# mueller-franzes/medfusion

Measured on AMD Instinct MI355X. Metric: images/sec at 256x256, 150 DDIM steps (DiffusionPipeline.sample incl. VAE decode), higher is better.
Workload: dtype f32 (emulated: fp16 pairs -- 23-bit operands, and 23-bit STORAGE of the tensors between the UNet's conv blocks: they exist as fp16 pairs only)

## Files before the change

medfusion_amd/csrc/conv_f16x2.hip:

```cpp
#include "common.h"
#include <string.h>
#include <mutex>
#include <vector>
#include "gn_partial.h"
#include "conv_plan.h"
#include "conv_f16x2.h"
#include "conv_f16x2_halo.h"
#include "conv_f16x2_group.h"
#include "winograd.h"

using namespace mf;

namespace {

struct Tile2 { int id, BM, BN, WM, WN, NST, HG; };
const Tile2 kTiles2[] = {
    {31, 128, 256, 2, 4, 3, 0}, {32, 256, 128, 4, 2, 3, 0}, {33, 128, 128, 2, 4, 3, 0}, {34, 128, 128, 4, 2, 3, 0}, {35, 256, 64, 4, 2, 3, 0},
    {36, 128, 64, 4, 2, 3, 0}, {37, 64, 256, 1, 8, 3, 0},
    {51, 128, 128, 2, 2, 2, 0}, {52, 128, 128, 2, 2, 3, 0}, {53, 64, 128, 2, 2, 3, 0}, {54, 128, 64, 2, 2, 3, 0},
    {61, 256, 128, 4, 2, 3, 6}, {62, 256, 128, 4, 2, 3, 7}, {63, 128, 128, 2, 4, 3, 4}, {64, 128, 128, 2, 4, 3, 5},
};
inline size_t tile_lds(const Tile2& t) {
  return t.HG ? (size_t)2 * t.HG * (t.WM * t.WN) * 1024 + (size_t)3 * t.BN * 128 : (size_t)t.NST * (t.BM + t.BN) * 128;
}
// ... 272 lines not shown
  if (pl.splitk > 1 && !(tree_possible(d, pl) && epilogue_stats_ok(d, pl, G)))
    return stats_lds_bytes(d->Cout / stats_slices(d->N, HW, d->Cout, G)) <= 64 * 1024 ? stats_chunks(HW) : 0;
  if (!epilogue_stats_ok(d, pl, G)) return 0;
  return HW >= pl.t.BM ? HW / pl.t.BM : 1;
}


}

namespace mf {
int f16x2_gn_parts(const MfConvDesc* d, int G) {
  Plan2 p2;
  return make_plan2(d, &p2) == MF_OK ? gn_parts2(d, p2, G) : 0;
}
size_t f16x2_workspace_bytes(const MfConvDesc* d) {
  Plan2 p2;
  if (make_plan2(d, &p2) != MF_OK || !p2.ok || p2.splitk <= 1) return 0;
  const size_t slabs = (size_t)p2.splitk * p2.M * d->Cout * sizeof(float);
  const size_t tree = tree_possible(d, p2) ? tree_handoff_bytes(d, p2) : 0;
  return slabs > tree ? slabs : tree;
}
}

#if MFC2_HZ & (256 | 512)
static float* g_conv_dbg = nullptr;
extern "C" void mf_debug_set_conv_dump(float* p) { g_conv_dbg = p; }
#endif

extern "C" {

int mf_conv2d_f16x2_ok(const MfConvDesc* d) {
  Plan2 pl;
  return d && pair_precision(d->precision) && make_plan2(d, &pl) == MF_OK && pl.ok ? 1 : 0;
}

static int bound_slots2(const MfConvDesc* d, const Plan2& pl, bool with_stats) {
  const int HW = pl.Hout * pl.Wout;
  if (pl.splitk == 1 || tree_possible(d, pl)) {
    if (!tile_sample_aligned(pl)) return 0;
    const int nw = pl.t.WM * pl.t.WN;
    return HW >= pl.t.BM ? (HW / pl.t.BM) * (d->Cout / pl.t.BN) * nw : (d->Cout / pl.t.BN) * (nw * HW / pl.t.BM);
  }
  if (with_stats) return 0;
  const long p4 = (long)HW * d->Cout / 4;
  int bx = (int)((p4 + 255) / 256);
  const int cap = cdiv(2048, d->N);
  if (bx > cap) bx = cap;
// ... 329 lines not shown
```

medfusion_amd/csrc/conv_f16x2_wino.inc:

```

static void wino_gemm_desc(const MfConvDesc* d, MfConvDesc* g) {
  *g = *d;
  g->N = 16 * d->N;
  g->Hin = 1;
  g->Win = (d->Hin / 2) * (d->Win / 2);
  g->KH = g->KW = 1;
  g->stride = 1;
  g->pad = 0;
  g->upsample = 3;
}
static bool wino_shape_ok(const MfConvDesc* d) {
  return d && d->precision == MF_CONV_FP32_F16X2 && d->KH == 3 && d->KW == 3 && d->stride == 1 && d->pad == 1 && d->upsample == 0 &&
         d->in_layout == MF_LAYOUT_NHWC && d->out_layout == MF_LAYOUT_NHWC && d->N > 0 && d->Hin >= 2 && d->Win >= 2 && d->Hin % 2 == 0 && d->Win % 2 == 0 &&
         d->C1 > 0 && d->C1 % 32 == 0 && d->C2 >= 0 && d->C2 % 32 == 0 && d->Cout % 64 == 0 && d->Cout <= 1024 && 256 % (d->Cout / 4) == 0 &&
         (double)d->N * 16.0 * (d->Hin / 2) * (d->Win / 2) < 2147483647.0;
}
static size_t wino_m_bytes(const MfConvDesc* d) {
  const size_t b = (size_t)16 * d->N * (d->Hin / 2) * (d->Win / 2) * d->Cout * sizeof(float);
  return (b + 255) & ~(size_t)255;
}
static bool wino_plan(const MfConvDesc* d, MfConvDesc* g, Plan2* pl) {
  if (!wino_shape_ok(d)) return false;
  wino_gemm_desc(d, g);
  if (make_plan2(g, pl) != MF_OK || !pl->ok) return false;
// ... 93 lines not shown
  const size_t mbytes = wino_m_bytes(d), need = mf_wino_workspace_bytes(d);
  MF_REQUIRE(workspace_bytes >= need, MF_EWORKSPACE, "conv_wino: workspace %zu < %zu", workspace_bytes, need);
  float* m = reinterpret_cast<float*>(workspace);
  int rc = conv_f16x2_prepare(v1s, v2s, us, nullptr, m, v1_bound, v2_bound, u_bound, nullptr, reinterpret_cast<char*>(workspace) + mbytes,
                              workspace_bytes - mbytes, sync, nullptr, 0, nullptr, &g, nullptr, &q, true);
  if (rc) return rc;
  MF_REQUIRE(q.pl.splitk == 1 || q.tree, MF_EUNSUPPORTED, "conv_wino: the component GEMM's split-K must meet inside the launch");
  hipStream_t s = (hipStream_t)stream;
  const int Cin = d->C1 + d->C2, T = (d->Hin / 2) * (d->Win / 2);
  const double M = (double)d->N * d->Hin * d->Win;
  {
    ProfScope ps(MF_FAM_CONV_IGEMM, s, 2.0 * M * d->Cout * 9.0 * Cin, 16.0 * M * Cin + 64.0 * d->Cout * Cin + 16.0 * M * d->Cout, 2.0 * 4.0 * M * d->Cout * Cin * 3.0);
    ps.set_tag(q.pl.t.id, 1);
    rc = dispatch_tile(q.pl.t.id, q.p, s, 3, 0);
    if (rc == -1) { set_error("conv_wino: no tile config %d", q.pl.t.id); rc = MF_EINVAL; }
  }
  if (rc) return rc;
  const int tpp = wino_tiles_per_part(d), parts = cdiv(T, tpp);
  ProfScope ps(MF_FAM_WINO_XFORM, s, 0, 4.0 * M * d->Cout * 5.0);
  MF_LAUNCH(mfw::wino_output_kernel, dim3(parts, d->N), dim3(256), 0, s, (const float*)m, bias, y, gn_partial, d->N, d->Hin, d->Win, d->Cout, G > 0 ? G : 1, tpp);
  return check_launch("wino_output");
}

int mf_wino_tail_ok(const MfConvDesc* d, int G) {
  if (!mf_wino_ok(d) || G <= 0 || d->Cout % G) return 0;
  const int cpg = d->Cout / G;
  if (cpg % 8 || 256 % (cpg / 4)) return 0;
  return (size_t)d->Hin * d->Win * cpg * sizeof(float) <= 64 * 1024 ? 1 : 0;
}

int mf_wino_group_ok(const MfConvDesc* d, const MfConvDesc* guest) {
  static const int off = [] { const char* e = getenv("MF_CONV_GROUP"); return e && atoi(e) == 0 ? 1 : 0; }();
  MfConvDesc g;
  Plan2 pl, pb;
  if (off || !guest || guest->precision != MF_CONV_FP32_F16X2 || !wino_plan(d, &g, &pl)) return 0;
  if (make_plan2(guest, &pb) != MF_OK || !pb.ok || !single_launch(guest, pb, 0)) return 0;
  mfc2::ConvP2 dummy{};
  return dispatch_group(pl.t.id, pb.t.id, dummy, dummy, nullptr, 2) == 1 ? 1 : 0;
}

int mf_conv2d_wino_gn_apply_f16x2(const void* v1s, const void* v2s, const void* us, const float* bias, const float* v1_bound, const float* v2_bound,
                                  float u_bound, void* workspace, size_t workspace_bytes, uint32_t* sync, int G, const MfWinoTail* t,
                                  const MfConvF16x2Call* guest, const MfConvDesc* d, void* stream) {
  MF_REQUIRE(d && t && v1s && us && workspace, MF_EINVAL, "conv_wino_gn_apply: null pointer");
  MF_REQUIRE(mf_wino_tail_ok(d, G), MF_EUNSUPPORTED, "conv_wino_gn_apply: not on this path (mf_wino_tail_ok == 0)");
  MF_REQUIRE(t->out || t->out_split || t->out_wino, MF_EINVAL, "conv_wino_gn_apply: no output");
  MF_REQUIRE(!(t->out_split || t->out_wino) || t->out_bound, MF_EINVAL, "conv_wino_gn_apply: out_bound with the fp16-pair outputs");
  MF_REQUIRE(!t->out_wino || t->wino_bound, MF_EINVAL, "conv_wino_gn_apply: wino_bound with out_wino");
  MF_REQUIRE((t->gamma == nullptr) == (t->beta == nullptr), MF_EINVAL, "conv_wino_gn_apply: gamma/beta must both be given or both NULL");
  MF_REQUIRE(!(t->residual && t->residual_pairs), MF_EINVAL, "conv_wino_gn_apply: the residual is fp32 OR fp16 pairs");
  MF_REQUIRE(!t->residual_pairs || t->res_bound, MF_EINVAL, "conv_wino_gn_apply: a residual given as fp16 pairs needs the res_bound that scaled it");
  MF_REQUIRE(!t->residual || t->res_bound || (t->res_bound_slots && t->res_nslots > 0), MF_EINVAL, "conv_wino_gn_apply: a residual needs res_bound or res_bound_slots");
  MF_REQUIRE(!t->emb || (t->emb_bound && t->emb_stride % 4 == 0), MF_EINVAL, "conv_wino_gn_apply: an embedding needs emb_bound and emb_stride %% 4 == 0");
  MfConvDesc g;
  Prep q;
  MF_REQUIRE(wino_plan(d, &g, &q.pl), MF_EUNSUPPORTED, "conv_wino_gn_apply: not on the Winograd path");
  const size_t mbytes = wino_m_bytes(d), need = mf_wino_workspace_bytes(d);
  MF_REQUIRE(workspace_bytes >= need, MF_EWORKSPACE, "conv_wino_gn_apply: workspace %zu < %zu", workspace_bytes, need);
  float* m = reinterpret_cast<float*>(workspace);
  int rc = conv_f16x2_prepare(v1s, v2s, us, nullptr, m, v1_bound, v2_bound, u_bound, nullptr, reinterpret_cast<char*>(workspace) + mbytes,
                              workspace_bytes - mbytes, sync, nullptr, 0, nullptr, &g, nullptr, &q, true);
  if (rc) return rc;
  MF_REQUIRE(q.pl.splitk == 1 || q.tree, MF_EUNSUPPORTED, "conv_wino_gn_apply: the component GEMM's split-K must meet inside the launch");
  hipStream_t s = (hipStream_t)stream;
  const int Cin = d->C1 + d->C2;
  const double M = (double)d->N * d->Hin * d->Win;
  const double gflops = 2.0 * M * d->Cout * 9.0 * Cin, gbytes = 16.0 * M * Cin + 64.0 * d->Cout * Cin + 16.0 * M * d->Cout , gexec = 2.0 * 4.0 * M * d->Cout * Cin * 3.0;
  if (guest) {
    MF_REQUIRE(guest->d && guest->y && mf_wino_group_ok(d, guest->d), MF_EUNSUPPORTED, "conv_wino_gn_apply: the guest cannot share this launch (mf_wino_group_ok == 0)");
    Prep qb;
    rc = conv_f16x2_prepare(guest->x1s, guest->x2s, guest->ws, guest->bias, guest->y, guest->x1_bound, guest->x2_bound, guest->w_bound, guest->y_bound,
                            guest->workspace, guest->workspace_bytes, guest->sync, guest->gn_partial, guest->G, nullptr, guest->d, nullptr, &qb);
    if (rc) return rc;
    MF_REQUIRE(qb.pl.splitk == 1 || qb.tree, MF_EUNSUPPORTED, "conv_wino_gn_apply: the guest's plan needs its reducer pass");
    if (qb.tree) {
      const char *wa = (const char*)workspace, *wb = (const char*)guest->workspace;
      MF_REQUIRE(wa + need <= wb || wb + tree_handoff_bytes(guest->d, qb.pl) <= wa, MF_EINVAL, "conv_wino_gn_apply: the guest's workspace overlaps the GEMM's");
      const long ca = mf_wino_sync_words(d), cb = mf_conv2d_f16x2_sync_words(guest->d);
      MF_REQUIRE(!sync || sync + ca <= guest->sync || guest->sync + cb <= sync, MF_EINVAL, "conv_wino_gn_apply: the guest's sync array overlaps the GEMM's");
    }
    MF_REQUIRE(guest->y != m, MF_EINVAL, "conv_wino_gn_apply: one output for two convolutions");
    ProfScope ps(MF_FAM_CONV_IGEMM, s, gflops + qb.flops, gbytes + qb.bytes, gexec + 2.0 * 3.0 * qb.pl.M * (double)guest->d->Cout * qb.pl.K);
    ps.set_tag(1000 + 100 * q.pl.t.id + qb.pl.t.id, 1);
    rc = dispatch_group(q.pl.t.id, qb.pl.t.id, q.p, qb.p, s, 0);
    if (rc == -1) { set_error("conv_wino_gn_apply: no tile pair (%d, %d)", q.pl.t.id, qb.pl.t.id); rc = MF_EINVAL; }
  } else {
    ProfScope ps(MF_FAM_CONV_IGEMM, s, gflops, gbytes, gexec);
    ps.set_tag(q.pl.t.id, 1);
    rc = dispatch_tile(q.pl.t.id, q.p, s, 3, 0);
    if (rc == -1) { set_error("conv_wino_gn_apply: no tile config %d", q.pl.t.id); rc = MF_EINVAL; }
  }
  if (rc) return rc;
  mfw::WinoTailP p;
  p.m = m; p.bias = bias; p.gamma = t->gamma; p.beta = t->beta;
  p.res_f32 = t->residual; p.res_pairs = t->residual_pairs; p.res_bound = t->res_bound; p.res_slots = t->res_bound ? nullptr : t->res_bound_slots;
  p.res_nslots = t->res_nslots; p.emb = t->emb; p.emb_stride = (long)t->emb_stride; p.emb_bound = t->emb_bound;
  p.out_f32 = t->out; p.out_pairs = t->out_split; p.out_bound = t->out_bound; p.out_wino = t->out_wino; p.wino_bound = t->wino_bound;
  p.N = d->N; p.H = d->Hin; p.W = d->Win; p.C = d->Cout; p.G = G; p.act = t->act; p.eps = t->eps; p.bconst = t->bconst;
  static const int v_nt = [] { const char* e = getenv("MF_WINO_VSTORE"); return e ? atoi(e) : 1; }();
  p.v_nt = v_nt;
  static const int tail_map = [] { const char* e = getenv("MF_WINO_TAIL_MAP"); return e ? atoi(e) : 1; }();
  p.xcd_map = tail_map;
  p.v_f32 = 0;
  const size_t lds = (size_t)d->Hin * d->Win * (d->Cout / G) * sizeof(float);
  {
    static DeviceOnce once;
    if (first_use_on_device(once)) (void)hipFuncSetAttribute(reinterpret_cast<const void*>(&mfw::wino_tail_kernel), hipFuncAttributeMaxDynamicSharedMemorySize, 64 * 1024);
  }
  ProfScope ps(MF_FAM_WINO_XFORM, s, 8.0 * M * d->Cout, 4.0 * M * d->Cout * (4 + (t->out ? 1 : 0) + (t->out_split ? 1 : 0) + (t->out_wino ? 4 : 0) + (t->residual || t->residual_pairs ? 1 : 0)));
  MF_LAUNCH(mfw::wino_tail_kernel, dim3((unsigned)G * (unsigned)d->N), dim3(256), lds, s, p);
  return check_launch("wino_tail");
}

int mf_wino_f32_ok(const MfConvDesc* d, int G) {
  if (!d || (d->precision != MF_CONV_FP32 && d->precision != MF_CONV_FP32_SPLIT3_W3) || d->KH != 3 || d->KW != 3 || d->stride != 1 || d->pad != 1 || d->upsample != 0 ||
      d->in_layout != MF_LAYOUT_NHWC || d->out_layout != MF_LAYOUT_NHWC || d->N <= 0 || d->Hin < 2 || d->Win < 2 || d->Hin % 2 || d->Win % 2 || d->C1 <= 0 || d->C1 % 32 ||
      d->C2 < 0 || d->C2 % 32 || d->Cout % 64 || d->Cout > 1024 || G <= 0 || d->Cout % G)
    return 0;
  const int cpg = d->Cout / G;
  if (cpg % 4 || 256 % (cpg / 4)) return 0;
  if ((size_t)d->Hin * d->Win * cpg * sizeof(float) > 64 * 1024) return 0;
  const long rows = (long)d->N * (d->Hin / 2) * (d->Win / 2);
  return rows % 64 == 0 && (double)rows * 16.0 < 2147483647.0 ? 1 : 0;
}

int mf_wino_input_f32(const float* x, float* v, int N, int H, int W, int C, void* stream) {
  MF_REQUIRE(x && v && N > 0 && H >= 2 && W >= 2 && H % 2 == 0 && W % 2 == 0 && C > 0 && C % 4 == 0, MF_EINVAL, "wino_input_f32: bad args (H, W even, C %% 4 == 0)");
  hipStream_t s = (hipStream_t)stream;
  const long total = (long)N * (H / 2) * (W / 2) * (C / 4);
  long blocks = (total + 255) / 256;
  if (blocks > 256 * 16) blocks = 256 * 16;
  ProfScope ps(MF_FAM_WINO_XFORM, s, 0, 4.0 * (double)N * H * W * C * 5.0);
  MF_LAUNCH(mfw::wino_input_f32_kernel, dim3((unsigned)blocks), dim3(256), 0, s, x, v, N, H, W, C);
  return check_launch("wino_input_f32");
}

int mf_wino_tail_f32(const float* m, const float* bias, const float* gamma, const float* beta, const float* residual, const float* emb, int64_t emb_stride,
                     float* out, float* out_wino, int N, int H, int W, int C, int G, int act, float eps, void* stream) {
  MF_REQUIRE(m && out && N > 0 && H >= 2 && W >= 2 && H % 2 == 0 && W % 2 == 0 && C > 0 && G > 0 && C % G == 0, MF_EINVAL, "wino_tail_f32: bad args");
  MF_REQUIRE((gamma == nullptr) == (beta == nullptr), MF_EINVAL, "wino_tail_f32: gamma/beta must both be given or both NULL");
  MF_REQUIRE(!emb || emb_stride % 4 == 0, MF_EINVAL, "wino_tail_f32: emb_stride %% 4 == 0");
  const int cpg = C / G;
  MF_REQUIRE(cpg % 4 == 0 && 256 % (cpg / 4) == 0, MF_EUNSUPPORTED, "wino_tail_f32: channels per group %d (a thread keeps its 4 channels)", cpg);
  const size_t lds = (size_t)H * W * cpg * sizeof(float);
  MF_REQUIRE(lds <= 64 * 1024, MF_EUNSUPPORTED, "wino_tail_f32: a sample's pixels x a group's channels do not fit in LDS (%zu bytes)", lds);
  hipStream_t s = (hipStream_t)stream;
  mfw::WinoTailP p;
  p.m = m; p.bias = bias; p.gamma = gamma; p.beta = beta;
  p.res_f32 = residual; p.res_pairs = nullptr; p.res_bound = nullptr; p.res_slots = nullptr; p.res_nslots = 0;
  p.emb = emb; p.emb_stride = (long)emb_stride; p.emb_bound = nullptr;
  p.out_f32 = out; p.out_pairs = nullptr; p.out_bound = nullptr; p.out_wino = out_wino; p.wino_bound = nullptr;
  p.N = N; p.H = H; p.W = W; p.C = C; p.G = G; p.act = act; p.eps = eps; p.bconst = 0.f;
  p.v_nt = 1; p.v_f32 = 1;
  static const int tail_map = [] { const char* e = getenv("MF_WINO_TAIL_MAP"); return e ? atoi(e) : 1; }();
  p.xcd_map = tail_map;
  {
    static DeviceOnce once;
    if (first_use_on_device(once)) (void)hipFuncSetAttribute(reinterpret_cast<const void*>(&mfw::wino_tail_kernel), hipFuncAttributeMaxDynamicSharedMemorySize, 64 * 1024);
  }
  const double M = (double)N * H * W;
  ProfScope ps(MF_FAM_WINO_XFORM, s, 8.0 * M * C, 4.0 * M * C * (4 + 1 + (out_wino ? 4 : 0) + (residual ? 1 : 0)));
  MF_LAUNCH(mfw::wino_tail_kernel, dim3((unsigned)G * (unsigned)N), dim3(256), lds, s, p);
  return check_launch("wino_tail_f32");
}

int mf_wino_plan_query(const MfConvDesc* d, int32_t* tile_id, int32_t* splitk) {
  MfConvDesc g;
  Plan2 pl;
  const bool ok = wino_plan(d, &g, &pl);
  if (tile_id) *tile_id = ok ? pl.t.id : 0;
  if (splitk) *splitk = ok ? pl.splitk : 0;
  return MF_OK;
}
```

medfusion_amd/csrc/winograd.h:

```cpp
#pragma once
#include "common.h"
#include "split_f16.h"

namespace mfw {
using namespace mf;
typedef float wf32x4 __attribute__((ext_vector_type(4)));

__global__ __launch_bounds__(256) void wino_pack_weight_kernel(const float* __restrict__ w, float* __restrict__ u, long n) {
  const long i = (long)blockIdx.x * 256 + threadIdx.x;
  if (i >= n) return;
  double g[3][3], t[4][3];
#pragma unroll
  for (int r = 0; r < 3; ++r)
#pragma unroll
    for (int c = 0; c < 3; ++c) g[r][c] = (double)w[i * 9 + r * 3 + c];
#pragma unroll
  for (int c = 0; c < 3; ++c) {
    t[0][c] = g[0][c];
    t[1][c] = 0.5 * (g[0][c] + g[1][c] + g[2][c]);
    t[2][c] = 0.5 * (g[0][c] - g[1][c] + g[2][c]);
    t[3][c] = g[2][c];
  }
#pragma unroll
  for (int r = 0; r < 4; ++r) {
// ... 162 lines not shown

struct WinoTailP {
  const float* m;
  const float* bias;
  const float* gamma;
  const float* beta;
  const float* res_f32;
  const void* res_pairs;
  const float* res_bound;
  const float* res_slots;
  int res_nslots;
  const float* emb;
  long emb_stride;
  const float* emb_bound;
  float* out_f32;
  void* out_pairs;
  float* out_bound;
  void* out_wino;
  float* wino_bound;
  int N, H, W, C, G, act;
  float eps, bconst;
  int v_nt;
  int v_f32;
  int xcd_map;
};

__device__ __forceinline__ float wino_pair_round(float a) {
  const _Float16 h = (_Float16)a;
  const _Float16 l = (_Float16)((a - (float)h) * kLoScale);
  return (float)h + (float)l * kLoInv;
}

__global__ __launch_bounds__(256) void wino_tail_kernel(const WinoTailP p) {
  extern __shared__ __attribute__((aligned(16))) float ys[];
  __shared__ double sd[8];
  __shared__ float sf[8];
  const int tid = threadIdx.x, lane = tid & 63, wave = tid >> 6;
  int lin = blockIdx.x;
  if (p.xcd_map) {
    const int total = p.G * p.N, q = total >> 3, r = total & 7, xcd = lin & 7, within = lin >> 3;
    lin = (xcd < r ? xcd * (q + 1) : r * (q + 1) + (xcd - r) * q) + within;
  }
  const int g = lin % p.G, n = lin / p.G;
  const int C = p.C, cpg = C / p.G, cq = cpg >> 2, c0 = g * cpg;
  const int H = p.H, W = p.W, HW = H * W, TW = W >> 1, T = (H >> 1) * TW;
  const long plane = (long)p.N * T * C;
  const int c4 = tid % cq;
  constexpr int RJ = 4;
  uint2 rph[RJ], rpl[RJ];
  float4 rpf[RJ];
#pragma unroll
  for (int j = 0; j < RJ; ++j) {
    rph[j] = make_uint2(0u, 0u); rpl[j] = make_uint2(0u, 0u); rpf[j] = make_float4(0.f, 0.f, 0.f, 0.f);
    const int it = tid + 256 * j;
    if (it < HW * cq) {
      const long eo = ((long)n * HW + it / cq) * C + c0 + c4 * 4;
      if (p.res_pairs) {
        const uint2* gp = reinterpret_cast<const uint2*>(reinterpret_cast<const char*>(p.res_pairs) + (eo >> 3) * 32 + ((eo >> 2) & 1) * 8);
        rph[j] = gp[0]; rpl[j] = gp[2];
      } else if (p.res_f32) {
        rpf[j] = *reinterpret_cast<const float4*>(p.res_f32 + eo);
      }
    }
  }
  const float4 b4 = p.bias ? *reinterpret_cast<const float4*>(p.bias + c0 + c4 * 4) : make_float4(0.f, 0.f, 0.f, 0.f);
  double s = 0, q = 0;
  for (int it = tid; it < T * cq; it += 256) {
    const int t = it / cq;
    const float* src = p.m + ((long)n * T + t) * C + c0 + c4 * 4;
    float4 v[16];
#pragma unroll
    for (int k = 0; k < 16; ++k) v[k] = *reinterpret_cast<const float4*>(src + (long)k * plane);
    float4 o[4];
#pragma unroll
    for (int e = 0; e < 4; ++e) {
      float mm[16];
#pragma unroll
      for (int k = 0; k < 16; ++k) mm[k] = e == 0 ? v[k].x : e == 1 ? v[k].y : e == 2 ? v[k].z : v[k].w;
      float a0[4], a1[4];
#pragma unroll
      for (int c = 0; c < 4; ++c) {
        a0[c] = (mm[c] + mm[4 + c]) + mm[8 + c];
        a1[c] = (mm[4 + c] - mm[8 + c]) - mm[12 + c];
      }
      const float be = e == 0 ? b4.x : e == 1 ? b4.y : e == 2 ? b4.z : b4.w;
      const float y00 = ((a0[0] + a0[1]) + a0[2]) + be, y01 = ((a0[1] - a0[2]) - a0[3]) + be;
      const float y10 = ((a1[0] + a1[1]) + a1[2]) + be, y11 = ((a1[1] - a1[2]) - a1[3]) + be;
      if (e == 0) { o[0].x = y00; o[1].x = y01; o[2].x = y10; o[3].x = y11; }
      if (e == 1) { o[0].y = y00; o[1].y = y01; o[2].y = y10; o[3].y = y11; }
      if (e == 2) { o[0].z = y00; o[1].z = y01; o[2].z = y10; o[3].z = y11; }
      if (e == 3) { o[0].w = y00; o[1].w = y01; o[2].w = y10; o[3].w = y11; }
    }
    const int ty = t / TW, tx = t - ty * TW;
    float* dst = ys + ((2 * ty) * W + 2 * tx) * cpg + c4 * 4;
    *reinterpret_cast<float4*>(dst) = o[0];
    *reinterpret_cast<float4*>(dst + cpg) = o[1];
    *reinterpret_cast<float4*>(dst + W * cpg) = o[2];
    *reinterpret_cast<float4*>(dst + W * cpg + cpg) = o[3];
    float s1 = 0.f, s2 = 0.f;
#pragma unroll
    for (int j = 0; j < 4; ++j) {
      s1 += (o[j].x + o[j].y) + (o[j].z + o[j].w);
      s2 = fmaf(o[j].x, o[j].x, s2); s2 = fmaf(o[j].y, o[j].y, s2); s2 = fmaf(o[j].z, o[j].z, s2); s2 = fmaf(o[j].w, o[j].w, s2);
    }
    s += (double)s1;
    q += (double)s2;
  }
#pragma unroll
  for (int off = 32; off > 0; off >>= 1) {
    s += __shfl_xor(s, off, 64);
    q += __shfl_xor(q, off, 64);
  }
  if (lane == 0) { sd[wave] = s; sd[4 + wave] = q; }
  if (p.res_slots) {
    float mx = 0.f;
    for (int i = tid; i < p.res_nslots; i += 256) mx = fmaxf(mx, p.res_slots[(long)n * p.res_nslots + i]);
    mx = wave_max(mx);
    if (lane == 0) sf[wave] = mx;
  }
  __syncthreads();
  const double S = ((sd[0] + sd[1]) + sd[2]) + sd[3], Q = ((sd[4] + sd[5]) + sd[6]) + sd[7];
  const double count = (double)HW * cpg;
  const double mean_d = S / count;
  double var = Q / count - mean_d * mean_d;
  if (var < 0) var = 0;
  const float mean = (float)mean_d, rstd = (float)(1.0 / sqrt(var + (double)p.eps));
  const float rb = p.res_slots ? fmaxf(fmaxf(sf[0], sf[1]), fmaxf(sf[2], sf[3])) : (p.res_bound ? p.res_bound[n] : 0.f);
  const float ob = p.bconst + rb + (p.emb_bound ? p.emb_bound[n] : 0.f);
  const float osc = exp2i(-scale_exp_of(ob));
  const float rsc = p.res_pairs ? exp2i(scale_exp_of(p.res_bound[n])) : 1.f;
  const float vb = 4.f * ob;
  if (g == 0) {
    if (tid == 0 && p.out_bound) p.out_bound[n] = ob;
    if (tid < 16 && p.wino_bound) p.wino_bound[tid * p.N + n] = vb;
  }
  float ga[4] = {1.f, 1.f, 1.f, 1.f}, be[4] = {0.f, 0.f, 0.f, 0.f};
  if (p.gamma) {
    const float4 g4 = *reinterpret_cast<const float4*>(p.gamma + c0 + c4 * 4), e4 = *reinterpret_cast<const float4*>(p.beta + c0 + c4 * 4);
    ga[0] = g4.x; ga[1] = g4.y; ga[2] = g4.z; ga[3] = g4.w;
    be[0] = e4.x; be[1] = e4.y; be[2] = e4.z; be[3] = e4.w;
  }
  const float4 em = p.emb ? *reinterpret_cast<const float4*>(p.emb + (long)n * p.emb_stride + c0 + c4 * 4) : make_float4(0.f, 0.f, 0.f, 0.f);
  const bool keep = p.out_wino != nullptr;
  auto pairs_to_f4 = [](uint2 h, uint2 l) {
    const sf_f16x2 h0 = __builtin_bit_cast(sf_f16x2, h.x), h1 = __builtin_bit_cast(sf_f16x2, h.y), l0 = __builtin_bit_cast(sf_f16x2, l.x),
                   l1 = __builtin_bit_cast(sf_f16x2, l.y);
    return make_float4((float)h0[0] + (float)l0[0] * kLoInv, (float)h0[1] + (float)l0[1] * kLoInv, (float)h1[0] + (float)l1[0] * kLoInv,
                       (float)h1[1] + (float)l1[1] * kLoInv);
  };
#define WINO_TAIL_ELEMENT(IT, RES_EXPR_PAIRS, RES_EXPR_F32)                                                            \
  {                                                                                                                   \
    const int pix = (IT) / cq;                                                                                        \
    float* yp = ys + pix * cpg + c4 * 4;                                                                              \
    const float4 v = *reinterpret_cast<const float4*>(yp);                                                            \
    float e[4] = {v.x, v.y, v.z, v.w};                                                                                \
    _Pragma("unroll") for (int k = 0; k < 4; ++k) {                                                                   \
      float t = (e[k] - mean) * rstd;                                                                                 \
      if (p.gamma) t = t * ga[k] + be[k];                                                                             \
      if (p.act == 1) t = swish_apply(t);                                                                             \
      e[k] = t;                                                                                                       \
    }                                                                                                                 \
    const long eo = ((long)n * HW + pix) * C + c0 + c4 * 4;                                                           \
    if (p.res_pairs) {                                                                                                \
      const float4 r = RES_EXPR_PAIRS;                                                                                \
      e[0] += r.x * rsc; e[1] += r.y * rsc; e[2] += r.z * rsc; e[3] += r.w * rsc;                                     \
    } else if (p.res_f32) {                                                                                           \
      const float4 r = RES_EXPR_F32;                                                                                  \
      e[0] += r.x; e[1] += r.y; e[2] += r.z; e[3] += r.w;                                                             \
    }                                                                                                                 \
    if (p.emb) { e[0] += em.x; e[1] += em.y; e[2] += em.z; e[3] += em.w; }                                            \
    if (p.out_f32) *reinterpret_cast<float4*>(p.out_f32 + eo) = make_float4(e[0], e[1], e[2], e[3]);                  \
    if (p.out_pairs) store_split4<false>(p.out_pairs, eo, e[0], e[1], e[2], e[3], osc);    \
    if (keep) *reinterpret_cast<float4*>(yp) = p.v_f32 ? make_float4(e[0], e[1], e[2], e[3])                                                                     \
                                                       : make_float4(wino_pair_round(e[0] * osc), wino_pair_round(e[1] * osc), wino_pair_round(e[2] * osc), wino_pair_round(e[3] * osc)); \
  }
#pragma unroll
  for (int j = 0; j < RJ; ++j) {
    const int it = tid + 256 * j;
    if (it < HW * cq) WINO_TAIL_ELEMENT(it, pairs_to_f4(rph[j], rpl[j]), rpf[j])
  }
  for (int it = tid + 256 * RJ; it < HW * cq; it += 256) WINO_TAIL_ELEMENT(it, wino_load_pairs4(p.res_pairs, eo), *reinterpret_cast<const float4*>(p.res_f32 + eo))
#undef WINO_TAIL_ELEMENT
  if (!keep) return;
  __syncthreads();
  const float f = exp2i(scale_exp_of(ob)) * exp2i(-scale_exp_of(vb));
  for (int it = tid; it < T * cq; it += 256) {
    const int t = it / cq, ty = t / TW, tx = t - ty * TW;
    float d[4][16];
#pragma unroll
    for (int py = 0; py < 4; ++py)
#pragma unroll
      for (int px = 0; px < 4; ++px) {
        const int y = 2 * ty - 1 + py, x = 2 * tx - 1 + px;
        float4 v = make_float4(0.f, 0.f, 0.f, 0.f);
        if ((unsigned)y < (unsigned)H && (unsigned)x < (unsigned)W) v = *reinterpret_cast<const float4*>(ys + (y * W + x) * cpg + c4 * 4);
        d[0][4 * py + px] = v.x; d[1][4 * py + px] = v.y; d[2][4 * py + px] = v.z; d[3][4 * py + px] = v.w;
      }
#pragma unroll
    for (int k = 0; k < 4; ++k) wino_bt_d_b(d[k]);
    const long e0 = ((long)n * T + t) * C + c0 + c4 * 4;
    if (p.v_f32) {
#pragma unroll
      for (int k = 0; k < 16; ++k)
        __builtin_nontemporal_store(wf32x4{d[0][k], d[1][k], d[2][k], d[3][k]}, reinterpret_cast<wf32x4*>(reinterpret_cast<float*>(p.out_wino) + (long)k * plane + e0));
    } else if (p.v_nt) {
#pragma unroll
      for (int k = 0; k < 16; ++k) store_split4<true, true>(p.out_wino, (long)k * plane + e0, d[0][k], d[1][k], d[2][k], d[3][k], f);
    } else {
#pragma unroll
      for (int k = 0; k < 16; ++k) store_split4<true>(p.out_wino, (long)k * plane + e0, d[0][k], d[1][k], d[2][k], d[3][k], f);
    }
  }
}

}
```

Measured before the change: 42.45.

## Restructure Winograd GN tail kernel with 32-bit offsets, pow2 indexing and DPP pair stores

```diff
diff --git a/medfusion_amd/csrc/conv_f16x2.hip b/medfusion_amd/csrc/conv_f16x2.hip
--- a/medfusion_amd/csrc/conv_f16x2.hip
+++ b/medfusion_amd/csrc/conv_f16x2.hip
@@ -318,7 +318,7 @@
 }
 }
 
-#if MFC2_HZ & (256 | 512)
+#if MFC2_HZ & (256 | 512 | 1024)
 static float* g_conv_dbg = nullptr;
 extern "C" void mf_debug_set_conv_dump(float* p) { g_conv_dbg = p; }
 #endif
diff --git a/medfusion_amd/csrc/conv_f16x2_wino.inc b/medfusion_amd/csrc/conv_f16x2_wino.inc
--- a/medfusion_amd/csrc/conv_f16x2_wino.inc
+++ b/medfusion_amd/csrc/conv_f16x2_wino.inc
@@ -139,10 +139,29 @@
   return check_launch("wino_output");
 }
 
+
+static bool wino_tail_offsets_ok(int N, int H, int W, int C) { return 16.0 * N * (H / 2) * (W / 2) * C * 4.0 < 4294967296.0; }
+
+static int wino_tail_launch(const mfw::WinoTailP& p, hipStream_t s, const char* what, bool general = false) {
+  const bool pow2 = !general && !(p.G & (p.G - 1)) && !((p.W >> 1) & ((p.W >> 1) - 1));
+  const size_t lds = (size_t)p.H * p.W * (p.C / p.G) * sizeof(float);
+  {
+    static DeviceOnce once;
+    if (first_use_on_device(once)) {
+      (void)hipFuncSetAttribute(reinterpret_cast<const void*>(&mfw::wino_tail_kernel<false>), hipFuncAttributeMaxDynamicSharedMemorySize, 64 * 1024);
+      (void)hipFuncSetAttribute(reinterpret_cast<const void*>(&mfw::wino_tail_kernel<true>), hipFuncAttributeMaxDynamicSharedMemorySize, 64 * 1024);
+    }
+  }
+  const dim3 grid((unsigned)p.G * (unsigned)p.N);
+  if (pow2) MF_LAUNCH(mfw::wino_tail_kernel<true>, grid, dim3(256), lds, s, p);
+  else MF_LAUNCH(mfw::wino_tail_kernel<false>, grid, dim3(256), lds, s, p);
+  return check_launch(what);
+}
 int mf_wino_tail_ok(const MfConvDesc* d, int G) {
   if (!mf_wino_ok(d) || G <= 0 || d->Cout % G) return 0;
   const int cpg = d->Cout / G;
   if (cpg % 8 || 256 % (cpg / 4)) return 0;
+  if (!wino_tail_offsets_ok(d->N, d->Hin, d->Win, d->Cout)) return 0;
   return (size_t)d->Hin * d->Win * cpg * sizeof(float) <= 64 * 1024 ? 1 : 0;
 }
 
@@ -156,11 +175,7 @@
   return dispatch_group(pl.t.id, pb.t.id, dummy, dummy, nullptr, 2) == 1 ? 1 : 0;
 }
 
-int mf_conv2d_wino_gn_apply_f16x2(const void* v1s, const void* v2s, const void* us, const float* bias, const float* v1_bound, const float* v2_bound,
-                                  float u_bound, void* workspace, size_t workspace_bytes, uint32_t* sync, int G, const MfWinoTail* t,
-                                  const MfConvF16x2Call* guest, const MfConvDesc* d, void* stream) {
-  MF_REQUIRE(d && t && v1s && us && workspace, MF_EINVAL, "conv_wino_gn_apply: null pointer");
-  MF_REQUIRE(mf_wino_tail_ok(d, G), MF_EUNSUPPORTED, "conv_wino_gn_apply: not on this path (mf_wino_tail_ok == 0)");
+static int wino_tail_check(const MfWinoTail* t) {
   MF_REQUIRE(t->out || t->out_split || t->out_wino, MF_EINVAL, "conv_wino_gn_apply: no output");
   MF_REQUIRE(!(t->out_split || t->out_wino) || t->out_bound, MF_EINVAL, "conv_wino_gn_apply: out_bound with the fp16-pair outputs");
   MF_REQUIRE(!t->out_wino || t->wino_bound, MF_EINVAL, "conv_wino_gn_apply: wino_bound with out_wino");
@@ -169,6 +184,41 @@
   MF_REQUIRE(!t->residual_pairs || t->res_bound, MF_EINVAL, "conv_wino_gn_apply: a residual given as fp16 pairs needs the res_bound that scaled it");
   MF_REQUIRE(!t->residual || t->res_bound || (t->res_bound_slots && t->res_nslots > 0), MF_EINVAL, "conv_wino_gn_apply: a residual needs res_bound or res_bound_slots");
   MF_REQUIRE(!t->emb || (t->emb_bound && t->emb_stride % 4 == 0), MF_EINVAL, "conv_wino_gn_apply: an embedding needs emb_bound and emb_stride %% 4 == 0");
+  return MF_OK;
+}
+static mfw::WinoTailP wino_tail_args(const float* m, const float* bias, const MfWinoTail* t, int N, int H, int W, int C, int G) {
+  mfw::WinoTailP p;
+  p.m = m; p.bias = bias; p.gamma = t->gamma; p.beta = t->beta;
+  p.res_f32 = t->residual; p.res_pairs = t->residual_pairs; p.res_bound = t->res_bound; p.res_slots = t->res_bound ? nullptr : t->res_bound_slots;
+  p.res_nslots = t->res_nslots; p.emb = t->emb; p.emb_stride = (long)t->emb_stride; p.emb_bound = t->emb_bound;
+  p.out_f32 = t->out; p.out_pairs = t->out_split; p.out_bound = t->out_bound; p.out_wino = t->out_wino; p.wino_bound = t->wino_bound;
+  p.N = N; p.H = H; p.W = W; p.C = C; p.G = G; p.act = t->act; p.eps = t->eps; p.bconst = t->bconst;
+  static const int v_nt = [] { const char* e = getenv("MF_WINO_VSTORE"); return e ? atoi(e) : 1; }();
+  p.v_nt = v_nt;
+  static const int tail_map = [] { const char* e = getenv("MF_WINO_TAIL_MAP"); return e ? atoi(e) : 1; }();
+  p.xcd_map = tail_map;
+#if MFC2_HZ & 1024
+  p.dbg = reinterpret_cast<unsigned long*>(g_conv_dbg);
+#endif
+  p.v_f32 = 0;
+  return p;
+}
+
+int mf_debug_wino_tail_f16x2(const float* m, const float* bias, int G, const MfWinoTail* t, int N, int H, int W, int C, int general, void* stream) {
+  MF_REQUIRE(m && t && N > 0 && H >= 2 && W >= 2 && H % 2 == 0 && W % 2 == 0 && C > 0 && G > 0 && C % G == 0, MF_EINVAL, "debug_wino_tail: bad args");
+  const int cpg = C / G;
+  MF_REQUIRE(cpg % 8 == 0 && 256 % (cpg / 4) == 0 && (size_t)H * W * cpg * sizeof(float) <= 64 * 1024 && wino_tail_offsets_ok(N, H, W, C), MF_EUNSUPPORTED,
+             "debug_wino_tail: not a shape of the tail (channels per group %d)", cpg);
+  if (int rc0 = wino_tail_check(t)) return rc0;
+  return wino_tail_launch(wino_tail_args(m, bias, t, N, H, W, C, G), (hipStream_t)stream, "wino_tail", general != 0);
+}
+
+int mf_conv2d_wino_gn_apply_f16x2(const void* v1s, const void* v2s, const void* us, const float* bias, const float* v1_bound, const float* v2_bound,
+                                  float u_bound, void* workspace, size_t workspace_bytes, uint32_t* sync, int G, const MfWinoTail* t,
+                                  const MfConvF16x2Call* guest, const MfConvDesc* d, void* stream) {
+  MF_REQUIRE(d && t && v1s && us && workspace, MF_EINVAL, "conv_wino_gn_apply: null pointer");
+  MF_REQUIRE(mf_wino_tail_ok(d, G), MF_EUNSUPPORTED, "conv_wino_gn_apply: not on this path (mf_wino_tail_ok == 0)");
+  if (int rc0 = wino_tail_check(t)) return rc0;
   MfConvDesc g;
   Prep q;
   MF_REQUIRE(wino_plan(d, &g, &q.pl), MF_EUNSUPPORTED, "conv_wino_gn_apply: not on the Winograd path");
@@ -208,25 +258,9 @@
     if (rc == -1) { set_error("conv_wino_gn_apply: no tile config %d", q.pl.t.id); rc = MF_EINVAL; }
   }
   if (rc) return rc;
-  mfw::WinoTailP p;
-  p.m = m; p.bias = bias; p.gamma = t->gamma; p.beta = t->beta;
-  p.res_f32 = t->residual; p.res_pairs = t->residual_pairs; p.res_bound = t->res_bound; p.res_slots = t->res_bound ? nullptr : t->res_bound_slots;
-  p.res_nslots = t->res_nslots; p.emb = t->emb; p.emb_stride = (long)t->emb_stride; p.emb_bound = t->emb_bound;
-  p.out_f32 = t->out; p.out_pairs = t->out_split; p.out_bound = t->out_bound; p.out_wino = t->out_wino; p.wino_bound = t->wino_bound;
-  p.N = d->N; p.H = d->Hin; p.W = d->Win; p.C = d->Cout; p.G = G; p.act = t->act; p.eps = t->eps; p.bconst = t->bconst;
-  static const int v_nt = [] { const char* e = getenv("MF_WINO_VSTORE"); return e ? atoi(e) : 1; }();
-  p.v_nt = v_nt;
-  static const int tail_map = [] { const char* e = getenv("MF_WINO_TAIL_MAP"); return e ? atoi(e) : 1; }();
-  p.xcd_map = tail_map;
-  p.v_f32 = 0;
-  const size_t lds = (size_t)d->Hin * d->Win * (d->Cout / G) * sizeof(float);
-  {
-    static DeviceOnce once;
-    if (first_use_on_device(once)) (void)hipFuncSetAttribute(reinterpret_cast<const void*>(&mfw::wino_tail_kernel), hipFuncAttributeMaxDynamicSharedMemorySize, 64 * 1024);
-  }
+  const mfw::WinoTailP p = wino_tail_args(m, bias, t, d->N, d->Hin, d->Win, d->Cout, G);
   ProfScope ps(MF_FAM_WINO_XFORM, s, 8.0 * M * d->Cout, 4.0 * M * d->Cout * (4 + (t->out ? 1 : 0) + (t->out_split ? 1 : 0) + (t->out_wino ? 4 : 0) + (t->residual || t->residual_pairs ? 1 : 0)));
-  MF_LAUNCH(mfw::wino_tail_kernel, dim3((unsigned)G * (unsigned)d->N), dim3(256), lds, s, p);
-  return check_launch("wino_tail");
+  return wino_tail_launch(p, s, "wino_tail");
 }
 
 int mf_wino_f32_ok(const MfConvDesc* d, int G) {
@@ -236,7 +270,7 @@
     return 0;
   const int cpg = d->Cout / G;
   if (cpg % 4 || 256 % (cpg / 4)) return 0;
-  if ((size_t)d->Hin * d->Win * cpg * sizeof(float) > 64 * 1024) return 0;
+  if ((size_t)d->Hin * d->Win * cpg * sizeof(float) > 64 * 1024 || !wino_tail_offsets_ok(d->N, d->Hin, d->Win, d->Cout)) return 0;
   const long rows = (long)d->N * (d->Hin / 2) * (d->Win / 2);
   return rows % 64 == 0 && (double)rows * 16.0 < 2147483647.0 ? 1 : 0;
 }
@@ -261,6 +295,7 @@
   MF_REQUIRE(cpg % 4 == 0 && 256 % (cpg / 4) == 0, MF_EUNSUPPORTED, "wino_tail_f32: channels per group %d (a thread keeps its 4 channels)", cpg);
   const size_t lds = (size_t)H * W * cpg * sizeof(float);
   MF_REQUIRE(lds <= 64 * 1024, MF_EUNSUPPORTED, "wino_tail_f32: a sample's pixels x a group's channels do not fit in LDS (%zu bytes)", lds);
+  MF_REQUIRE(wino_tail_offsets_ok(N, H, W, C), MF_EUNSUPPORTED, "wino_tail_f32: M exceeds 4 GB");
   hipStream_t s = (hipStream_t)stream;
   mfw::WinoTailP p;
   p.m = m; p.bias = bias; p.gamma = gamma; p.beta = beta;
@@ -269,16 +304,14 @@
   p.out_f32 = out; p.out_pairs = nullptr; p.out_bound = nullptr; p.out_wino = out_wino; p.wino_bound = nullptr;
   p.N = N; p.H = H; p.W = W; p.C = C; p.G = G; p.act = act; p.eps = eps; p.bconst = 0.f;
   p.v_nt = 1; p.v_f32 = 1;
+#if MFC2_HZ & 1024
+  p.dbg = nullptr;
+#endif
   static const int tail_map = [] { const char* e = getenv("MF_WINO_TAIL_MAP"); return e ? atoi(e) : 1; }();
   p.xcd_map = tail_map;
-  {
-    static DeviceOnce once;
-    if (first_use_on_device(once)) (void)hipFuncSetAttribute(reinterpret_cast<const void*>(&mfw::wino_tail_kernel), hipFuncAttributeMaxDynamicSharedMemorySize, 64 * 1024);
-  }
   const double M = (double)N * H * W;
   ProfScope ps(MF_FAM_WINO_XFORM, s, 8.0 * M * C, 4.0 * M * C * (4 + 1 + (out_wino ? 4 : 0) + (residual ? 1 : 0)));
-  MF_LAUNCH(mfw::wino_tail_kernel, dim3((unsigned)G * (unsigned)N), dim3(256), lds, s, p);
-  return check_launch("wino_tail_f32");
+  return wino_tail_launch(p, s, "wino_tail_f32");
 }
 
 int mf_wino_plan_query(const MfConvDesc* d, int32_t* tile_id, int32_t* splitk) {
diff --git a/medfusion_amd/csrc/winograd.h b/medfusion_amd/csrc/winograd.h
--- a/medfusion_amd/csrc/winograd.h
+++ b/medfusion_amd/csrc/winograd.h
@@ -208,6 +208,9 @@
   float eps, bconst;
   int v_nt;
   int v_f32;
+#if MFC2_HZ & 1024
+  unsigned long* dbg;
+#endif
   int xcd_map;
 };
 
@@ -217,67 +220,139 @@
   return (float)h + (float)l * kLoInv;
 }
 
+template <bool CLAMP, bool NT>
+__device__ __forceinline__ void wino_store_split4(char* base, unsigned off, bool odd, float a, float b, float c, float d, float sc) {
+  unsigned h0, h1, l0, l1;
+  split2_f16<CLAMP>(a * sc, b * sc, h0, l0);
+  split2_f16<CLAMP>(c * sc, d * sc, h1, l1);
+  const unsigned s0 = odd ? h0 : l0, s1 = odd ? h1 : l1;
+  const unsigned r0 = (unsigned)__builtin_amdgcn_mov_dpp((int)s0, 0xB1, 0xF, 0xF, true);
+  const unsigned r1 = (unsigned)__builtin_amdgcn_mov_dpp((int)s1, 0xB1, 0xF, 0xF, true);
+  const sf_u32x4 v = odd ? sf_u32x4{r0, r1, l0, l1} : sf_u32x4{h0, h1, r0, r1};
+  sf_u32x4* q = reinterpret_cast<sf_u32x4*>(base + (size_t)off);
+  if (NT) __builtin_nontemporal_store(v, q);
+  else *q = v;
+}
+
+__device__ __forceinline__ void wino_at_m_a(const float4 (&v)[16], const float4 b4, float4 (&o)[4]) {
+#pragma unroll
+  for (int e = 0; e < 4; ++e) {
+    float mm[16];
+#pragma unroll
+    for (int k = 0; k < 16; ++k) mm[k] = e == 0 ? v[k].x : e == 1 ? v[k].y : e == 2 ? v[k].z : v[k].w;
+    float a0[4], a1[4];
+#pragma unroll
+    for (int c = 0; c < 4; ++c) {
+      a0[c] = (mm[c] + mm[4 + c]) + mm[8 + c];
+      a1[c] = (mm[4 + c] - mm[8 + c]) - mm[12 + c];
+    }
+    const float be = e == 0 ? b4.x : e == 1 ? b4.y : e == 2 ? b4.z : b4.w;
+    const float y00 = ((a0[0] + a0[1]) + a0[2]) + be, y01 = ((a0[1] - a0[2]) - a0[3]) + be;
+    const float y10 = ((a1[0] + a1[1]) + a1[2]) + be, y11 = ((a1[1] - a1[2]) - a1[3]) + be;
+    if (e == 0) { o[0].x = y00; o[1].x = y01; o[2].x = y10; o[3].x = y11; }
+    if (e == 1) { o[0].y = y00; o[1].y = y01; o[2].y = y10; o[3].y = y11; }
+    if (e == 2) { o[0].z = y00; o[1].z = y01; o[2].z = y10; o[3].z = y11; }
+    if (e == 3) { o[0].w = y00; o[1].w = y01; o[2].w = y10; o[3].w = y11; }
+  }
+}
+
+struct WinoTailPair {
+  int g, n, c0;
+  float4 b4, g4, e4, em;
+  float rb, eb, rsc;
+};
+template <bool POW2>
+__device__ __forceinline__ WinoTailPair wino_tail_pair(const WinoTailP& p, int lin, int gsh, int cpg, int c4) {
+  WinoTailPair c;
+  c.g = POW2 ? lin & (p.G - 1) : lin % p.G;
+  c.n = POW2 ? lin >> gsh : lin / p.G;
+  c.c0 = c.g * cpg;
+  const int ch = c.c0 + c4 * 4;
+  c.b4 = c.e4 = c.em = make_float4(0.f, 0.f, 0.f, 0.f);
+  c.g4 = make_float4(1.f, 1.f, 1.f, 1.f);
+  c.rb = c.eb = 0.f;
+  c.rsc = 1.f;
+  if (p.bias) c.b4 = *reinterpret_cast<const float4*>(p.bias + ch);
+  if (p.gamma) {
+    c.g4 = *reinterpret_cast<const float4*>(p.gamma + ch);
+    c.e4 = *reinterpret_cast<const float4*>(p.beta + ch);
+  }
+  if (p.emb) c.em = *reinterpret_cast<const float4*>(p.emb + (long)c.n * p.emb_stride + ch);
+  if (p.res_bound) c.rb = p.res_bound[c.n];
+  if (p.emb_bound) c.eb = p.emb_bound[c.n];
+  if (p.res_pairs) c.rsc = exp2i(scale_exp_of(c.rb));
+  return c;
+}
+
+#if MFC2_HZ & 1024
+#define WINO_STAMP(I) { if (p.dbg && threadIdx.x == 0) p.dbg[(long)blockIdx.x * 8 + (I)] = __builtin_amdgcn_s_memrealtime(); }
+#else
+#define WINO_STAMP(I)
+#endif
+
+template <bool POW2>
 __global__ __launch_bounds__(256) void wino_tail_kernel(const WinoTailP p) {
   extern __shared__ __attribute__((aligned(16))) float ys[];
   __shared__ double sd[8];
-  __shared__ float sf[8];
+  __shared__ float sf[4];
   const int tid = threadIdx.x, lane = tid & 63, wave = tid >> 6;
+  WINO_STAMP(0)
+  const int C = p.C, H = p.H, W = p.W, HW = H * W, TW = W >> 1, T = (H >> 1) * TW;
+  const int gsh = POW2 ? __builtin_ctz(p.G) : 0, twsh = POW2 ? __builtin_ctz(TW) : 0;
+  const int cpg = POW2 ? C >> gsh : C / p.G, cq = cpg >> 2, cqs = __builtin_ctz(cq);
   int lin = blockIdx.x;
   if (p.xcd_map) {
     const int total = p.G * p.N, q = total >> 3, r = total & 7, xcd = lin & 7, within = lin >> 3;
     lin = (xcd < r ? xcd * (q + 1) : r * (q + 1) + (xcd - r) * q) + within;
   }
-  const int g = lin % p.G, n = lin / p.G;
-  const int C = p.C, cpg = C / p.G, cq = cpg >> 2, c0 = g * cpg;
-  const int H = p.H, W = p.W, HW = H * W, TW = W >> 1, T = (H >> 1) * TW;
-  const long plane = (long)p.N * T * C;
-  const int c4 = tid % cq;
+  const int c4 = tid & (cq - 1), pix0 = tid >> cqs, pstep = 256 >> cqs;
+  const bool odd = c4 & 1;
+  const unsigned eoff0 = (unsigned)(pix0 * C + c4 * 4), estep = (unsigned)(pstep * C);
+  const unsigned proff0 = (unsigned)(pix0 * C) * 4u + (unsigned)(c4 >> 1) * 32u + (odd ? 8u : 0u);
+  const int items1 = T << cqs, items2 = HW << cqs;
+  const unsigned plane4 = (unsigned)p.N * (unsigned)T * (unsigned)C * 4u;
+  const bool keep = p.out_wino != nullptr;
   constexpr int RJ = 4;
-  uint2 rph[RJ], rpl[RJ];
-  float4 rpf[RJ];
-#pragma unroll
-  for (int j = 0; j < RJ; ++j) {
-    rph[j] = make_uint2(0u, 0u); rpl[j] = make_uint2(0u, 0u); rpf[j] = make_float4(0.f, 0.f, 0.f, 0.f);
-    const int it = tid + 256 * j;
-    if (it < HW * cq) {
-      const long eo = ((long)n * HW + it / cq) * C + c0 + c4 * 4;
-      if (p.res_pairs) {
-        const uint2* gp = reinterpret_cast<const uint2*>(reinterpret_cast<const char*>(p.res_pairs) + (eo >> 3) * 32 + ((eo >> 2) & 1) * 8);
-        rph[j] = gp[0]; rpl[j] = gp[2];
-      } else if (p.res_f32) {
-        rpf[j] = *reinterpret_cast<const float4*>(p.res_f32 + eo);
-      }
-    }
-  }
-  const float4 b4 = p.bias ? *reinterpret_cast<const float4*>(p.bias + c0 + c4 * 4) : make_float4(0.f, 0.f, 0.f, 0.f);
+
+  auto load_m = [&](float4(&v)[16], int n, int c0, unsigned eoff) {
+    const char* mb = reinterpret_cast<const char*>(p.m + ((long)n * T * C + c0));
+#pragma unroll
+    for (int k = 0; k < 16; ++k) v[k] = *reinterpret_cast<const float4*>(mb + (size_t)(eoff * 4u + (unsigned)k * plane4));
+  };
+  auto load_res = [&](uint4(&rp)[RJ], int n, int c0) {
+    const long eu = (long)n * HW * C + c0;
+#pragma unroll
+    for (int j = 0; j < RJ; ++j) {
+      rp[j] = make_uint4(0u, 0u, 0u, 0u);
+      if (tid + 256 * j < items2) {
+        if (p.res_pairs) {
+          const uint2* gp = reinterpret_cast<const uint2*>(reinterpret_cast<const char*>(p.res_pairs) + eu * 4 + (size_t)(proff0 + (unsigned)j * estep * 4u));
+          const uint2 h = gp[0], l = gp[2];
+          rp[j] = make_uint4(h.x, h.y, l.x, l.y);
+        } else if (p.res_f32) {
+          rp[j] = *reinterpret_cast<const uint4*>(reinterpret_cast<const char*>(p.res_f32) + eu * 4 + (size_t)((eoff0 + (unsigned)j * estep) * 4u));
+        }
+      }
+    }
+  };
+  auto pairs_to_f4 = [](uint4 r) {
+    const sf_f16x2 h0 = __builtin_bit_cast(sf_f16x2, r.x), h1 = __builtin_bit_cast(sf_f16x2, r.y), l0 = __builtin_bit_cast(sf_f16x2, r.z),
+                   l1 = __builtin_bit_cast(sf_f16x2, r.w);
+    return make_float4((float)h0[0] + (float)l0[0] * kLoInv, (float)h0[1] + (float)l0[1] * kLoInv, (float)h1[0] + (float)l1[0] * kLoInv,
+                       (float)h1[1] + (float)l1[1] * kLoInv);
+  };
+
+  float4 v[16];
+  uint4 rp[RJ];
+  const WinoTailPair pc = wino_tail_pair<POW2>(p, lin, gsh, cpg, c4);
+  const int n = pc.n, c0 = pc.c0;
+  load_res(rp, n, c0);
+  if (tid < items1) load_m(v, n, c0, eoff0);
   double s = 0, q = 0;
-  for (int it = tid; it < T * cq; it += 256) {
-    const int t = it / cq;
-    const float* src = p.m + ((long)n * T + t) * C + c0 + c4 * 4;
-    float4 v[16];
-#pragma unroll
-    for (int k = 0; k < 16; ++k) v[k] = *reinterpret_cast<const float4*>(src + (long)k * plane);
+  auto phase1 = [&](int t) {
     float4 o[4];
-#pragma unroll
-    for (int e = 0; e < 4; ++e) {
-      float mm[16];
-#pragma unroll
-      for (int k = 0; k < 16; ++k) mm[k] = e == 0 ? v[k].x : e == 1 ? v[k].y : e == 2 ? v[k].z : v[k].w;
-      float a0[4], a1[4];
-#pragma unroll
-      for (int c = 0; c < 4; ++c) {
-        a0[c] = (mm[c] + mm[4 + c]) + mm[8 + c];
-        a1[c] = (mm[4 + c] - mm[8 + c]) - mm[12 + c];
-      }
-      const float be = e == 0 ? b4.x : e == 1 ? b4.y : e == 2 ? b4.z : b4.w;
-      const float y00 = ((a0[0] + a0[1]) + a0[2]) + be, y01 = ((a0[1] - a0[2]) - a0[3]) + be;
-      const float y10 = ((a1[0] + a1[1]) + a1[2]) + be, y11 = ((a1[1] - a1[2]) - a1[3]) + be;
-      if (e == 0) { o[0].x = y00; o[1].x = y01; o[2].x = y10; o[3].x = y11; }
-      if (e == 1) { o[0].y = y00; o[1].y = y01; o[2].y = y10; o[3].y = y11; }
-      if (e == 2) { o[0].z = y00; o[1].z = y01; o[2].z = y10; o[3].z = y11; }
-      if (e == 3) { o[0].w = y00; o[1].w = y01; o[2].w = y10; o[3].w = y11; }
-    }
-    const int ty = t / TW, tx = t - ty * TW;
+    wino_at_m_a(v, pc.b4, o);
+    const int ty = POW2 ? t >> twsh : t / TW, tx = POW2 ? t & (TW - 1) : t - ty * TW;
     float* dst = ys + ((2 * ty) * W + 2 * tx) * cpg + c4 * 4;
     *reinterpret_cast<float4*>(dst) = o[0];
     *reinterpret_cast<float4*>(dst + cpg) = o[1];
@@ -291,7 +366,18 @@
     }
     s += (double)s1;
     q += (double)s2;
-  }
+  };
+  if (tid < items1) phase1(pix0);
+  {
+    int t = pix0 + pstep;
+    unsigned eoff = eoff0 + estep;
+    for (int it = tid + 256; it < items1; it += 256, t += pstep, eoff += estep) {
+      asm volatile("" : "+v"(eoff));
+      load_m(v, n, c0, eoff);
+      phase1(t);
+    }
+  }
+  WINO_STAMP(1)
 #pragma unroll
   for (int off = 32; off > 0; off >>= 1) {
     s += __shfl_xor(s, off, 64);
@@ -305,48 +391,38 @@
     if (lane == 0) sf[wave] = mx;
   }
   __syncthreads();
+  WINO_STAMP(2)
   const double S = ((sd[0] + sd[1]) + sd[2]) + sd[3], Q = ((sd[4] + sd[5]) + sd[6]) + sd[7];
   const double count = (double)HW * cpg;
   const double mean_d = S / count;
   double var = Q / count - mean_d * mean_d;
   if (var < 0) var = 0;
   const float mean = (float)mean_d, rstd = (float)(1.0 / sqrt(var + (double)p.eps));
-  const float rb = p.res_slots ? fmaxf(fmaxf(sf[0], sf[1]), fmaxf(sf[2], sf[3])) : (p.res_bound ? p.res_bound[n] : 0.f);
-  const float ob = p.bconst + rb + (p.emb_bound ? p.emb_bound[n] : 0.f);
+  const float rb = p.res_slots ? fmaxf(fmaxf(sf[0], sf[1]), fmaxf(sf[2], sf[3])) : pc.rb;
+  const float ob = p.bconst + rb + pc.eb;
   const float osc = exp2i(-scale_exp_of(ob));
-  const float rsc = p.res_pairs ? exp2i(scale_exp_of(p.res_bound[n])) : 1.f;
+  const float rsc = pc.rsc;
   const float vb = 4.f * ob;
-  if (g == 0) {
+  if (pc.g == 0) {
     if (tid == 0 && p.out_bound) p.out_bound[n] = ob;
     if (tid < 16 && p.wino_bound) p.wino_bound[tid * p.N + n] = vb;
   }
-  float ga[4] = {1.f, 1.f, 1.f, 1.f}, be[4] = {0.f, 0.f, 0.f, 0.f};
-  if (p.gamma) {
-    const float4 g4 = *reinterpret_cast<const float4*>(p.gamma + c0 + c4 * 4), e4 = *reinterpret_cast<const float4*>(p.beta + c0 + c4 * 4);
-    ga[0] = g4.x; ga[1] = g4.y; ga[2] = g4.z; ga[3] = g4.w;
-    be[0] = e4.x; be[1] = e4.y; be[2] = e4.z; be[3] = e4.w;
-  }
-  const float4 em = p.emb ? *reinterpret_cast<const float4*>(p.emb + (long)n * p.emb_stride + c0 + c4 * 4) : make_float4(0.f, 0.f, 0.f, 0.f);
-  const bool keep = p.out_wino != nullptr;
-  auto pairs_to_f4 = [](uint2 h, uint2 l) {
-    const sf_f16x2 h0 = __builtin_bit_cast(sf_f16x2, h.x), h1 = __builtin_bit_cast(sf_f16x2, h.y), l0 = __builtin_bit_cast(sf_f16x2, l.x),
-                   l1 = __builtin_bit_cast(sf_f16x2, l.y);
-    return make_float4((float)h0[0] + (float)l0[0] * kLoInv, (float)h0[1] + (float)l0[1] * kLoInv, (float)h1[0] + (float)l1[0] * kLoInv,
-                       (float)h1[1] + (float)l1[1] * kLoInv);
-  };
-#define WINO_TAIL_ELEMENT(IT, RES_EXPR_PAIRS, RES_EXPR_F32)                                                            \
+  const float ga[4] = {pc.g4.x, pc.g4.y, pc.g4.z, pc.g4.w}, be[4] = {pc.e4.x, pc.e4.y, pc.e4.z, pc.e4.w};
+  const float4 em = pc.em;
+  const long eu = (long)n * HW * C + c0;
+  char* const of32 = reinterpret_cast<char*>(p.out_f32) + eu * 4;
+  char* const opairs = reinterpret_cast<char*>(p.out_pairs) + eu * 4;
+#define WINO_TAIL_ELEMENT(IT, EOFF, RES_EXPR_PAIRS, RES_EXPR_F32)                                                      \
   {                                                                                                                   \
-    const int pix = (IT) / cq;                                                                                        \
-    float* yp = ys + pix * cpg + c4 * 4;                                                                              \
-    const float4 v = *reinterpret_cast<const float4*>(yp);                                                            \
-    float e[4] = {v.x, v.y, v.z, v.w};                                                                                \
+    float* yp = ys + (IT) * 4;                                   \
+    const float4 v4 = *reinterpret_cast<const float4*>(yp);                                                           \
+    float e[4] = {v4.x, v4.y, v4.z, v4.w};                                                                            \
     _Pragma("unroll") for (int k = 0; k < 4; ++k) {                                                                   \
       float t = (e[k] - mean) * rstd;                                                                                 \
       if (p.gamma) t = t * ga[k] + be[k];                                                                             \
       if (p.act == 1) t = swish_apply(t);                                                                             \
       e[k] = t;                                                                                                       \
     }                                                                                                                 \
-    const long eo = ((long)n * HW + pix) * C + c0 + c4 * 4;                                                           \
     if (p.res_pairs) {                                                                                                \
       const float4 r = RES_EXPR_PAIRS;                                                                                \
       e[0] += r.x * rsc; e[1] += r.y * rsc; e[2] += r.z * rsc; e[3] += r.w * rsc;                                     \
@@ -355,48 +431,66 @@
       e[0] += r.x; e[1] += r.y; e[2] += r.z; e[3] += r.w;                                                             \
     }                                                                                                                 \
     if (p.emb) { e[0] += em.x; e[1] += em.y; e[2] += em.z; e[3] += em.w; }                                            \
-    if (p.out_f32) *reinterpret_cast<float4*>(p.out_f32 + eo) = make_float4(e[0], e[1], e[2], e[3]);                  \
-    if (p.out_pairs) store_split4<false>(p.out_pairs, eo, e[0], e[1], e[2], e[3], osc);    \
+    if (p.out_f32) *reinterpret_cast<float4*>(of32 + (size_t)((EOFF) * 4u)) = make_float4(e[0], e[1], e[2], e[3]);    \
+    if (p.out_pairs) wino_store_split4<false, false>(opairs, (EOFF) * 4u, odd, e[0], e[1], e[2], e[3], osc);    \
     if (keep) *reinterpret_cast<float4*>(yp) = p.v_f32 ? make_float4(e[0], e[1], e[2], e[3])                                                                     \
                                                        : make_float4(wino_pair_round(e[0] * osc), wino_pair_round(e[1] * osc), wino_pair_round(e[2] * osc), wino_pair_round(e[3] * osc)); \
   }
 #pragma unroll
   for (int j = 0; j < RJ; ++j) {
     const int it = tid + 256 * j;
-    if (it < HW * cq) WINO_TAIL_ELEMENT(it, pairs_to_f4(rph[j], rpl[j]), rpf[j])
-  }
-  for (int it = tid + 256 * RJ; it < HW * cq; it += 256) WINO_TAIL_ELEMENT(it, wino_load_pairs4(p.res_pairs, eo), *reinterpret_cast<const float4*>(p.res_f32 + eo))
+    const unsigned eoff = eoff0 + (unsigned)j * estep;
+    if (it < items2) WINO_TAIL_ELEMENT(it, eoff, pairs_to_f4(rp[j]), __builtin_bit_cast(float4, rp[j]))
+  }
+  {
+    unsigned eoff = eoff0 + RJ * estep, proff = proff0 + RJ * estep * 4u;
+    for (int it = tid + 256 * RJ; it < items2; it += 256, eoff += estep, proff += estep * 4u) {
+      asm volatile("" : "+v"(eoff), "+v"(proff));
+      const char* rq = reinterpret_cast<const char*>(p.res_pairs) + eu * 4 + (size_t)proff;
+      WINO_TAIL_ELEMENT(it, eoff, pairs_to_f4(make_uint4(reinterpret_cast<const uint2*>(rq)[0].x, reinterpret_cast<const uint2*>(rq)[0].y, reinterpret_cast<const uint2*>(rq)[2].x, reinterpret_cast<const uint2*>(rq)[2].y)),
+                        *reinterpret_cast<const float4*>(reinterpret_cast<const char*>(p.res_f32) + eu * 4 + (size_t)(eoff * 4u)))
+    }
+  }
 #undef WINO_TAIL_ELEMENT
-  if (!keep) return;
-  __syncthreads();
-  const float f = exp2i(scale_exp_of(ob)) * exp2i(-scale_exp_of(vb));
-  for (int it = tid; it < T * cq; it += 256) {
-    const int t = it / cq, ty = t / TW, tx = t - ty * TW;
-    float d[4][16];
-#pragma unroll
-    for (int py = 0; py < 4; ++py)
-#pragma unroll
-      for (int px = 0; px < 4; ++px) {
-        const int y = 2 * ty - 1 + py, x = 2 * tx - 1 + px;
-        float4 v = make_float4(0.f, 0.f, 0.f, 0.f);
-        if ((unsigned)y < (unsigned)H && (unsigned)x < (unsigned)W) v = *reinterpret_cast<const float4*>(ys + (y * W + x) * cpg + c4 * 4);
-        d[0][4 * py + px] = v.x; d[1][4 * py + px] = v.y; d[2][4 * py + px] = v.z; d[3][4 * py + px] = v.w;
-      }
-#pragma unroll
-    for (int k = 0; k < 4; ++k) wino_bt_d_b(d[k]);
-    const long e0 = ((long)n * T + t) * C + c0 + c4 * 4;
-    if (p.v_f32) {
-#pragma unroll
-      for (int k = 0; k < 16; ++k)
-        __builtin_nontemporal_store(wf32x4{d[0][k], d[1][k], d[2][k], d[3][k]}, reinterpret_cast<wf32x4*>(reinterpret_cast<float*>(p.out_wino) + (long)k * plane + e0));
-    } else if (p.v_nt) {
-#pragma unroll
-      for (int k = 0; k < 16; ++k) store_split4<true, true>(p.out_wino, (long)k * plane + e0, d[0][k], d[1][k], d[2][k], d[3][k], f);
-    } else {
-#pragma unroll
-      for (int k = 0; k < 16; ++k) store_split4<true>(p.out_wino, (long)k * plane + e0, d[0][k], d[1][k], d[2][k], d[3][k], f);
-    }
-  }
-}
-
-}
+  if (keep) {
+    __syncthreads();
+    const float f = exp2i(scale_exp_of(ob)) * exp2i(-scale_exp_of(vb));
+    char* const ov = reinterpret_cast<char*>(p.out_wino) + ((long)n * T * C + c0) * 4;
+    int t = pix0;
+    unsigned eoff = eoff0;
+    for (int it = tid; it < items1; it += 256, t += pstep, eoff += estep) {
+      asm volatile("" : "+v"(eoff));
+      const int ty = POW2 ? t >> twsh : t / TW, tx = POW2 ? t & (TW - 1) : t - ty * TW;
+      float d[4][16];
+#pragma unroll
+      for (int py = 0; py < 4; ++py)
+#pragma unroll
+        for (int px = 0; px < 4; ++px) {
+          const int y = 2 * ty - 1 + py, x = 2 * tx - 1 + px;
+          float4 u = make_float4(0.f, 0.f, 0.f, 0.f);
+          if ((unsigned)y < (unsigned)H && (unsigned)x < (unsigned)W) u = *reinterpret_cast<const float4*>(ys + (y * W + x) * cpg + c4 * 4);
+          d[0][4 * py + px] = u.x; d[1][4 * py + px] = u.y; d[2][4 * py + px] = u.z; d[3][4 * py + px] = u.w;
+        }
+#pragma unroll
+      for (int k = 0; k < 4; ++k) wino_bt_d_b(d[k]);
+      if (p.v_f32) {
+#pragma unroll
+        for (int k = 0; k < 16; ++k)
+          __builtin_nontemporal_store(wf32x4{d[0][k], d[1][k], d[2][k], d[3][k]}, reinterpret_cast<wf32x4*>(ov + (size_t)(eoff * 4u + (unsigned)k * plane4)));
+      } else if (p.v_nt) {
+#pragma unroll
+        for (int k = 0; k < 16; ++k) wino_store_split4<true, true>(ov, eoff * 4u + (unsigned)k * plane4, odd, d[0][k], d[1][k], d[2][k], d[3][k], f);
+      } else {
+#pragma unroll
+        for (int k = 0; k < 16; ++k) wino_store_split4<true, false>(ov, eoff * 4u + (unsigned)k * plane4, odd, d[0][k], d[1][k], d[2][k], d[3][k], f);
+      }
+    }
+  }
+  WINO_STAMP(3)
+#if MFC2_HZ & 1024
+  asm volatile("s_waitcnt vmcnt(0)" ::: "memory");
+#endif
+  WINO_STAMP(4)
+}
+
+}
```

Result: no change. 42.74, median of 6 (+0.7%).
